# pyranha-labs/hypergrep

Measured on AMD Instinct MI355X. Metric: GiB/s scanned (256 patterns, 32 GiB synthetic log per GPU, text resident in HBM), higher is better.
Workload: dtype u8

## Files before the change

__graft_entry__.py:

```python
from __future__ import annotations

import os
import subprocess
import sys

REPO = os.path.dirname(os.path.abspath(__file__))
if REPO not in sys.path:
    sys.path.insert(0, REPO)


def build() -> None:
    try:
        import torch
    except ImportError:
        pass
    from hypergrep_amd import build as native

    native.build(verbose=bool(os.environ.get("HG_VERBOSE")))
    subprocess.check_call(["make", "-C", os.path.join(REPO, "oracle")], stdout=subprocess.DEVNULL)
    sys.path.insert(0, os.path.join(REPO, "tests"))
    import hgsim_py

    hgsim_py.build()
    import hypergrep_amd

    assert hypergrep_amd.check_compatibility(["foobar"]) == 0


def smoke() -> None:
    import torch

    sys.path.insert(0, os.path.join(REPO, "tests"))
    import oracle_py
    from hypergrep_amd import benchspec, device

    assert torch.cuda.is_available(), "smoke() needs a GPU"
    patterns, needles, hpm = benchspec.c3_spec()
    nbytes = 4 << 20
# ... 20 lines not shown
```

hypergrep_amd/csrc/hg_compile.cpp:

```cpp
#include "hg_compile.h"
#include "hg_comb.h"
#include "hg_core.h"

#include <algorithm>
#include <array>
#include <bitset>
#include <cmath>
#include <cstdlib>
#include <cstring>
#include <map>
#include <memory>
#include <stdexcept>
#include <unordered_map>

namespace {

using ByteSet = std::bitset<256>;

constexpr int kThisExpression = -2;
struct CompileError : std::runtime_error {
  int index;
  explicit CompileError(const std::string &what, int index = kThisExpression) : std::runtime_error(what), index(index) {}
};

// ... 931 lines not shown
Lit clip(const Lit &l, size_t *offset = nullptr) {
  if (offset) *offset = 0;
  if (l.bytes.size() <= HG_FACTOR_MAX) return l;
  size_t best = 0;
  int best_score = INT32_MAX;
  for (size_t o = 0; o + HG_FACTOR_MAX <= l.bytes.size(); o++) {
    int s = 0;
    for (size_t i = 0; i < HG_FACTOR_MAX; i++) s += byte_commonness(static_cast<unsigned char>(l.bytes[o + i]));
    if (s < best_score) { best_score = s; best = o; }
  }
  if (offset) *offset = best;
  return {l.bytes.substr(best, HG_FACTOR_MAX), l.cmask.substr(best, HG_FACTOR_MAX)};
}

struct SampleStats {
  std::unordered_map<uint32_t, uint32_t> c4;
  std::unordered_map<uint64_t, uint32_t> c6;
  size_t dwords = 0;
};

int build_filter(HgDb &db, const SampleStats *stats, std::string *err) {
  db.windows.clear();
  std::vector<std::pair<uint32_t, HgWindow>> keyed;
  std::vector<uint32_t> next16_of;
  const uint32_t fold = db.fold_mask;
  const uint32_t wbytes = db.window_bytes, wmask = db.window_mask;
  std::unordered_map<uint32_t, uint32_t> contenders;
  for (uint32_t fi = 0; fi < db.nreal_factors; fi++) {
    const HgFactor &fct = db.factors[fi];
    std::vector<uint32_t> mine;
// ... 226 lines not shown
        if (rate < k_rate) { k_rate = rate; k_w = weights; }
      }
      if (k_rate < best_rate) { best_rate = k_rate; best_k = k; best_w = k_w; }
      if (k_rate <= (k <= 12 ? 5e-4 : 3e-4)) {
        best_rate = k_rate;
        best_k = k;
        best_w = k_w;
        placed = true;
      }
    }
    if (!placed && best_k && best_rate <= 2e-3 && values.size() * 100 <= (size_t(1) << HG_FILTER_MAX_LOG2) * 45) placed = true;
    if (placed) {
      const uint32_t k = best_k, wa = best_w;
      const uint32_t byte_mask = ((1u << k) - 1u) << 2;
      slot_words(k, wa, db.filter);
      db.ext.assign(size_t(1) << k, HgSlotInfo{});
      db.filter_log2 = k;
      db.weights_a = wa;
      db.weights_b = wa;
      auto merge = [](uint32_t &val, uint32_t &mask, uint32_t v2, uint32_t m2) {
        uint32_t keep = 0;
        for (int b = 0; b < 4; b++) {
          uint32_t bm = 0xFFu << (8 * b);
          if ((mask & bm) && (m2 & bm) && ((val ^ v2) & bm) == 0) keep |= bm;
        }
        mask = keep;
        val &= keep;
      };
      for (size_t wi = 0; wi < keyed.size(); wi++) {
        const HgWindow &w = keyed[wi].second;
// ... 69 lines not shown
      for (size_t e = 0; e < entries.size() && placed; e++) {
        int32_t cur = static_cast<int32_t>(e);
        bool ok = false;
        for (int kick = 0; kick < 8000 && !ok; kick++) {
          const uint32_t cand[4] = {entries[cur].sa * 2, entries[cur].sa * 2 + 1, entries[cur].sb * 2, entries[cur].sb * 2 + 1};
          for (uint32_t cell : cand)
            if (owner[cell] < 0) { owner[cell] = cur; ok = true; break; }
          if (ok) break;
          rng = rng * 6364136223846793005ull + 1442695040888963407ull;
          std::swap(cur, owner[cand[(rng >> 33) & 3]]);
        }
        if (!ok) placed = false;
      }
      if (!placed) continue;
      db.filter.assign(size_t(1) << k, HG_FILTER_EMPTY);
      for (size_t cell = 0; cell < cells; cell++) {
        if (owner[cell] < 0) continue;
        uint32_t &word = db.filter[cell >> 1];
        const uint32_t fp = entries[owner[cell]].fp;
        word = (cell & 1) ? ((word & 0x0000FFFFu) | (fp << 16)) : ((word & 0xFFFF0000u) | fp);
      }
      db.ext.assign(1, HgSlotInfo{});
      db.filter_log2 = k;
      db.filter_wide = 1;
      db.weights_a = wa;
      db.weights_b = wb;
    }
  }
  if (!placed) {
    if (err) *err = "too many distinct literal windows for the LDS filter (more than ~55 000)";
// ... 867 lines not shown
int hgc_tune(const HgDb *db, const uint8_t *sample, size_t nbytes, HgDb **out, std::string *err) {
  if (out) *out = nullptr;
  if (!db || !out || (!sample && nbytes)) return -1;
  SampleStats st;
  const uint32_t fold = db->fold_mask;
  for (size_t p = 0; p + 4 <= nbytes; p += db->dense ? db->dense : 4) {
    uint32_t w, nx = 0;
    std::memcpy(&w, sample + p, 4);
    if (p + 8 <= nbytes) std::memcpy(&nx, sample + p + 4, 4);
    w = (w | fold) & db->window_mask;
    nx |= fold;
    st.c4[w]++;
    st.c6[static_cast<uint64_t>(w) | (static_cast<uint64_t>(nx & 0xFFFFu) << 32)]++;
  }
  st.dwords = nbytes / 4;
  std::unique_ptr<HgDb> copy;
  try {
    copy = std::make_unique<HgDb>(*db);
  } catch (const std::bad_alloc &) {
    if (err) *err = "out of memory";
    return -2;
  }
  int rc = build_filter(*copy, &st, err);
  if (rc != 0) return rc;
  copy->tuned = true;
  *out = copy.release();
  return 0;
}

void hgc_free(HgDb *db) { delete db; }
// ... 1 lines not shown
```

hypergrep_amd/csrc/hg_compile.h:

```cpp
#pragma once
#include <cstdint>
#include <string>
#include <vector>

#include "../../include/hypergrep_amd.h"
#include "hg_core.h"
#include "hg_db.h"

struct HgDb {
  std::vector<HgPattern> patterns;
  std::vector<uint32_t> pool;
  std::vector<HgFactor> factors;
  uint32_t nreal_factors = 0;
  std::vector<HgWindow> windows;
  std::vector<uint32_t> bucket_off;
  std::vector<uint16_t> disc;
  std::vector<uint32_t> bucket_off2;
  std::vector<HgWindow> windows2;
  std::vector<HgWinBucket> wtab;
  uint32_t wtab_mask = 0;
  uint32_t shared_windows = 0;
  uint32_t wtab_first = 0;
  std::vector<uint32_t> filter;
  uint32_t filter_log2 = HG_FILTER_MIN_LOG2;
  uint32_t filter_wide = 0;
  uint32_t window_bytes = HG_WINDOW_BYTES;
  uint32_t window_mask = HG_WINDOW_MASK;
  uint32_t weights_c = HG_HASH_WEIGHTS;
  uint32_t dense = 0;
  uint32_t weights_a = HG_SLOT_WEIGHT_CHOICES[0][0], weights_b = HG_SLOT_WEIGHT_CHOICES[0][1];
  std::vector<HgSlotInfo> ext;
  std::vector<uint32_t> slow;
  uint32_t nslow_fast = 0;
  std::vector<HgSlowGroup> groups;
  uint32_t nslow_grouped = 0;
  uint32_t fold_mask = 0;
  uint32_t max_nw = 1;
  uint32_t nhuge = 0;
// ... 26 lines not shown
```

hypergrep_amd/csrc/hg_db.h:

```cpp
#pragma once
#include <cstdint>

#if defined(__HIPCC__)
#define HG_HD __host__ __device__ __forceinline__
#else
#define HG_HD inline
#endif

constexpr uint32_t HG_FLAG_CASELESS = 1, HG_FLAG_DOTALL = 2, HG_FLAG_MULTILINE = 4, HG_FLAG_SINGLEMATCH = 8;
constexpr uint32_t HG_FLAG_SOM_LEFTMOST = 256;
constexpr uint32_t HG_FLAG_COMBINATION = 512, HG_FLAG_QUIET = 1024;
constexpr uint32_t HG_FLAGS_SUPPORTED = 15 | HG_FLAG_SOM_LEFTMOST | HG_FLAG_COMBINATION | HG_FLAG_QUIET;

enum : uint32_t { HG_PC_START = 0, HG_PC_NL = 1, HG_PC_WORD = 2, HG_PC_OTHER = 3 };
enum : uint32_t { HG_NC_NL = 0, HG_NC_NLFINAL = 1, HG_NC_WORD = 2, HG_NC_OTHER = 3, HG_NC_END = 4 };
constexpr uint32_t HG_TT_ALL = (1u << 20) - 1;

constexpr uint32_t HG_MAX_NODES = 1024;
constexpr uint32_t HG_MAX_W = HG_MAX_NODES / 32;
constexpr uint32_t HG_HUGE_MAX_PROGRAM = 400000;
constexpr uint32_t HG_HUGE_MAX_NODES = 1u << 19;
constexpr uint32_t HG_HUGE_STAGE_MAX = 12288;
constexpr uint32_t HG_HUGE_MAX_EDGES = 1u << 22;
constexpr uint32_t HG_MAX_PATTERNS = 1u << 24;
// ... 127 lines not shown
  uint32_t ctx_off;
  uint32_t reserved;
};
static_assert(sizeof(HgSlowGroup) == 104, "HgSlowGroup layout");

HG_HD uint32_t hg_dot4(uint32_t v, uint32_t w) {
#if defined(__HIP_DEVICE_COMPILE__)
  return __builtin_amdgcn_udot4(v, w, 0u, false);
#else
  return (v & 0xff) * (w & 0xff) + ((v >> 8) & 0xff) * ((w >> 8) & 0xff) + ((v >> 16) & 0xff) * ((w >> 16) & 0xff) + (v >> 24) * (w >> 24);
#endif
}
HG_HD uint32_t hg_hash_window(uint32_t folded) { return hg_dot4(folded, HG_HASH_WEIGHTS); }
HG_HD uint32_t hg_slot(uint32_t folded, uint32_t weights, uint32_t byte_mask) { return hg_dot4(folded, weights) & byte_mask; }
HG_HD bool hg_slot_match(uint32_t slot_word, uint32_t hash_c) { return (hash_c & (slot_word >> 16)) == (slot_word & 0xFFFFu); }
HG_HD uint32_t hg_slot_wide(uint32_t sum_x, uint32_t sum_y, uint32_t byte_mask) { return (sum_x + (sum_y << 8)) & byte_mask; }

struct HgFilterExt {
  uint32_t pv, pm;
  uint32_t nv, nm;
};
HG_HD bool hg_ext_pass(const HgFilterExt &e, uint32_t prev_folded, uint32_t next_folded) {
  return (((prev_folded ^ e.pv) & e.pm) | ((next_folded ^ e.nv) & e.nm)) == 0;
}

constexpr uint32_t HG_DISC_WEIGHTS_1 = 0xc5a36b1du, HG_DISC_WEIGHTS_2 = 0x3b9d47e1u;
HG_HD uint32_t hg_disc_bytes(uint32_t sel4) {
  return ((sel4 & 1u) ? 0xFFu : 0u) | ((sel4 & 2u) ? 0xFF00u : 0u) | ((sel4 & 4u) ? 0xFF0000u : 0u) | ((sel4 & 8u) ? 0xFF000000u : 0u);
}
HG_HD uint32_t hg_disc_bucket(uint32_t h, uint32_t masked_dword) {
// ... 26 lines not shown
```

hypergrep_amd/csrc/hg_engine.h:

```cpp
#pragma once
#include <hip/hip_runtime.h>

#include <memory>
#include <string>

#include "../../include/hypergrep_amd.h"
#include "hg_compile.h"
#include "hg_core.h"
#include "hg_invert.h"
#include "hg_post.h"

#ifndef HG_STREAM_WG_WAVES
#define HG_STREAM_WG_WAVES 8
#endif
constexpr uint32_t HG_STREAM_WG_WAVES_DEFAULT = HG_STREAM_WG_WAVES;

constexpr uint32_t HG_CONFIRM_SPLIT = 4;
constexpr uint32_t HG_DEFER_SHARDS = 64;

struct HgDeferred {
  uint64_t pos;
  uint32_t pattern;
  uint32_t rank;
};
enum { HG_ST_MINLEN_KEPT = 16, HG_ST_FIN_TOTAL = 24, HG_ST_SELECTED = 28, HG_ST_FINAL = 32, HG_ST_WORDS = 36, HG_ST_ZERO_WORDS = 32,
       HG_ST_BLOCK_DONE = 40 };
enum { HG_CNT_CANDS = 0, HG_CNT_HITS = 1, HG_CNT_CAND_NEED = 2, HG_CNT_HIT_NEED = 3, HG_CNT_DEFER_NEED = 4,
       HG_CNT_HITS_WRAPPED = 5,
       HG_CNT_JOIN_TILES = 6,
       HG_CNT_WORDS = 8,
       HG_CNT_CURSOR0 = 64,
       HG_CNT_CURSORS = 64,
       HG_ST_ALLOC_WORDS = 128 };
constexpr uint32_t HG_STREAM_GRAB = 2 * HG_STREAM_WG_WAVES_DEFAULT;

constexpr uint32_t HG_FIN_MAX_BUCKETS = 1u << 22;
constexpr uint32_t HG_FIN_BUCKET_CAP = 4096;
constexpr uint32_t HG_FIN_MEDIUM_CAP = 512;

#ifndef HG_CONFIRM_THREADS
#define HG_CONFIRM_THREADS 128
#endif



// ... 237 lines not shown
```

hypergrep_amd/csrc/hg_engine.hip:

```cpp
#include <algorithm>
#include <array>
#include <cstdio>
#include <cstdlib>
#include <cstring>
#include <memory>

#include "hg_engine.h"
#include "hg_mem.h"

#include <rocprim/rocprim.hpp>

bool hg_launch_stream(const HgStreamArgs &a, uint32_t grid, hipStream_t stream);
bool hg_launch_stream_join(const HgStreamArgs &a, uint32_t grid, hipStream_t stream);
int hg_stream_blocks_per_cu(uint32_t filter_log2, uint32_t filter_wide, uint32_t dense);
__global__ void hg_tile_reduce_kernel(const HgTileSum *sums, uint64_t tile_begin, uint64_t tile_end, uint64_t bs1, HgTileElem *agg);
__global__ void hg_tile_spine_kernel(const HgTileElem *agg, uint32_t nblocks, uint64_t bs1, HgTileBase *block_base, HgTileBase *state);
__global__ void hg_tile_apply_kernel(const HgTileSum *sums, uint64_t tile_begin, uint64_t tile_end, uint64_t bs1, const HgTileBase *block_base,
                                     HgTileBase *bases);
__global__ void hg_tile_inner_kernel(const uint8_t *text, HgTileSum *sums, uint64_t tile_begin, uint64_t tile_end, uint64_t bs1);
__global__ void hg_verify_kernel(HgConfirmArgs a);
__global__ void hg_confirm_fast_kernel(HgConfirmArgs a, uint32_t blocks_per_mode);
__global__ void hg_confirm_generic_kernel(HgConfirmArgs a);
__global__ void hg_always_on_kernel(HgConfirmArgs a, uint32_t first, uint32_t last);
__global__ void hg_always_on_fast_kernel(HgConfirmArgs a);
// ... 118 lines not shown
  knobs_ = HgEngineKnobs::from_env();
  const HgDb &db = *db_;
  HG_TRY(hipSetDevice(device_), "hipSetDevice");
  hipDeviceProp_t prop;
  HG_TRY(hipGetDeviceProperties(&prop, device_), "hipGetDeviceProperties");
  num_cus_ = prop.multiProcessorCount;
  HG_TRY(upload(&d_patterns_, db.patterns, "d_patterns_"), "upload patterns");
  HG_TRY(upload(&d_pool_, db.pool, "d_pool_"), "upload tables");
  HG_TRY(upload(&d_factors_, db.factors, "d_factors_"), "upload factors");
  HG_TRY(upload(&d_windows_, db.windows, "d_windows_"), "upload windows");
  HG_TRY(upload(&d_bucket_, db.bucket_off, "d_bucket_"), "upload buckets");
  HG_TRY(upload(&d_disc_, db.disc, "d_disc_"), "upload discriminators");
  HG_TRY(upload(&d_bucket2_, db.bucket_off2, "d_bucket2_"), "upload buckets");
  HG_TRY(upload(&d_windows2_, db.windows2, "d_windows2_"), "upload windows");
  HG_TRY(upload(&d_wtab_, db.wtab, "d_wtab_"), "upload window table");
  HG_TRY(upload(&d_filter_, db.filter, "d_filter_"), "upload filter");
  HG_TRY(upload(&d_ext_, db.ext, "d_ext_"), "upload filter conditions");
  HG_TRY(upload(&d_slow_, db.slow, "d_slow_"), "upload always-on list");
  HG_TRY(upload(&d_groups_, db.groups, "d_groups_"), "upload always-on groups");
  view_.patterns = static_cast<const HgPattern *>(d_patterns_);
  view_.pool = static_cast<const uint32_t *>(d_pool_);
  view_.factors = static_cast<const HgFactor *>(d_factors_);
  view_.windows = static_cast<const HgWindow *>(d_windows_);
  view_.bucket_off = static_cast<const uint32_t *>(d_bucket_);
  view_.disc = static_cast<const uint16_t *>(d_disc_);
  view_.bucket_off2 = static_cast<const uint32_t *>(d_bucket2_);
  view_.windows2 = static_cast<const HgWindow *>(d_windows2_);
  view_.wtab = static_cast<const HgWinBucket *>(d_wtab_);
  view_.wtab_mask = db.wtab_mask;
  view_.wtab_first = db.wtab_first;
  view_.slow = static_cast<const uint32_t *>(d_slow_);
// ... 214 lines not shown
    p.wgs_alone = knobs_.stream_wgs_per_cu ? p.wgs_shared : grid_for(static_cast<uint32_t>(stream_wgs_per_cu_));
    p.joiner_wgs = (p.piped && stream_wgs_per_cu_ >= 3 && per_cu < static_cast<uint32_t>(stream_wgs_per_cu_) && chunk_limit_tiles_ == 0 && !side_bound_) ? static_cast<uint32_t>(num_cus_) : 0u;
    if (knobs_.joiner >= 0) p.joiner_wgs = p.piped ? static_cast<uint32_t>(knobs_.joiner) * static_cast<uint32_t>(num_cus_) : 0u;
    if (p.wgs_shared + p.joiner_wgs > max_segs_ || db_->filter_wide || db_->filter_log2 > 13) p.joiner_wgs = 0;
    p.wgs = std::max(p.wgs_shared + p.joiner_wgs, p.wgs_alone);
    for (uint32_t c = 0; c < std::min(nchunks, 2u); c++)
      p.cand_seg_cap[c] = static_cast<uint32_t>(static_cast<uint64_t>(cand_cap_) * 4 / (4ull * p.wgs_of(c) + p.joiners_of(c)));
  }
  HgStreamArgs &sa = p.sa;
  sa.text = text;
  sa.nbytes = nbytes;
  sa.db = view_;
  sa.filter = static_cast<const uint32_t *>(d_filter_);
  sa.filter_log2 = db_->filter_log2;
  sa.weights_a = db_->weights_a;
  sa.weights_b = db_->weights_b;
  sa.filter_wide = db_->filter_wide;
  sa.dense = db_->dense;
  sa.weights_c = db_->weights_c;
  sa.ext = static_cast<const HgSlotInfo *>(d_ext_);
  sa.sums = d_sums_;
  sa.counters = d_counters_;
  HgConfirmArgs &ca = p.ca;
  ca.text = text;
  ca.nbytes = nbytes;
  ca.bs1 = bs1;
  ca.db = view_;
  ca.sums = d_sums_;
  ca.bases = d_bases_;
  ca.hits = d_hits_raw_;
  ca.aux = d_aux_raw_;
// ... 437 lines not shown
  HG_TRY(hipMemcpyAsync(h_counters_, d_counters_, HG_ST_WORDS * 4, hipMemcpyDeviceToHost, stream), "copy state");
  if (p.bucketed) HG_TRY(hipEventRecord(ev_[3], stream), "event");
  HG_TRY(hipStreamSynchronize(stream), "stream sync (scan kernels)");
  if (p.piped) {
    uint32_t late = 0;
    for (uint32_t c = 0; c < p.nchunks; c++) {
      float ms = 0;
      (void)hipEventElapsedTime(&ms, ev_k1_begin_[c], ev_k1_end_[c]);
      out->ms_stream += ms;
      if (c >= 1 && hipEventElapsedTime(&ms, ev_k1_end_[c], ev_side_done_[c - 1]) == hipSuccess && ms > 0) late++;
    }
    side_bound_ = late * 2 > p.nchunks - 1;
  }

  out->joiner_tiles = h_counters_[HG_CNT_JOIN_TILES];
  const uint64_t n_raw = p.bucketed ? h_counters_[HG_ST_FIN_TOTAL + 1] : h_counters_[HG_CNT_HITS];
  if (int rc = regrow(p, n_raw)) return rc;
  fin_expect_hits_ = n_raw;
  const uint64_t n_pieces = block_mode ? 1 : !range.last ? 0 : h_final_->L - line_base + (nbytes > h_final_->cs ? hg_pieces(nbytes - h_final_->cs, bs1) : 0);
  uint32_t n = static_cast<uint32_t>(n_raw);
  const HgHit *fin_hits = d_hits_raw_;
  const HgHitAux *fin_aux = d_aux_raw_;
  if (n && d_min_lengths_) {
    if (int rc = minlen_pass(text, &n, p.stream)) return rc;
    fin_hits = d_minlen_hits_;
    fin_aux = d_minlen_aux_;
  }
  if (n && !p.bucketed)
    if (int rc = finalize_compact(fin_hits, fin_aux, n, p.id_bits, p.to_bits, line_base + (range.last ? n_pieces : nbytes) + 1, p.stream)) return rc;
  if (!p.bucketed) {
// ... 150 lines not shown
```

hypergrep_amd/csrc/hg_stream.hip:

```cpp
#include <hip/hip_runtime.h>
#include <cstdlib>

#include "hg_core.h"
#include "hg_engine.h"

namespace {

constexpr int WG_WAVES = HG_STREAM_WG_WAVES;
constexpr int WG_THREADS = WG_WAVES * 64;
constexpr int ITERS = HG_TILE_BYTES / 1024;

__device__ __forceinline__ uint32_t wave_inclusive_scan(uint32_t v, uint32_t lane) {
#pragma unroll
  for (int o = 1; o < 64; o <<= 1) {
    uint32_t u = __shfl_up(v, o, 64);
    if (lane >= static_cast<uint32_t>(o)) v += u;
  }
  return v;
}

}

namespace {

// ... 15 lines not shown
using lds_u32 = __attribute__((address_space(3))) uint32_t;

constexpr uint32_t queue_cap(int) { return 128u; }
constexpr bool queue_stash(int log2, bool dense) { return log2 <= 12 && !dense; }
constexpr uint32_t queue_entry_dw(int log2, bool dense) { return queue_stash(log2, dense) ? 8u : 2u; }
__device__ __forceinline__ uint32_t queue_chunk(uint32_t e0) { return e0 >> 16; }
__device__ __forceinline__ uint32_t queue_rank(uint32_t e0) { return e0 & 0xFFFFu; }

template <int LOG2, bool WIDE>
struct Probe {
  static constexpr uint32_t BYTE_MASK = ((1u << LOG2) - 1u) << 2;
  __device__ __forceinline__ static uint32_t at(const lds_u32 *filter, uint32_t byte_off) {
    return *reinterpret_cast<const lds_u32 *>(reinterpret_cast<const __attribute__((address_space(3))) uint8_t *>(filter) + byte_off);
  }
  template <bool ANY_ONLY, bool FOLD = true>
  __device__ __forceinline__ static uint32_t probe4(const lds_u32 *filter, uint32_t fold, uint32_t wa, uint32_t wb, uint4 v) {
    const uint32_t f0 = FOLD ? v.x | fold : v.x, f1 = FOLD ? v.y | fold : v.y, f2 = FOLD ? v.z | fold : v.z, f3 = FOLD ? v.w | fold : v.w;
    const uint32_t a0 = hg_dot4(f0, wa), a1 = hg_dot4(f1, wa), a2 = hg_dot4(f2, wa), a3 = hg_dot4(f3, wa);
    const uint32_t b0 = hg_dot4(f0, wb), b1 = hg_dot4(f1, wb), b2 = hg_dot4(f2, wb), b3 = hg_dot4(f3, wb);
    const uint32_t c0 = hg_dot4(f0, HG_HASH_WEIGHTS), c1 = hg_dot4(f1, HG_HASH_WEIGHTS);
    const uint32_t c2 = hg_dot4(f2, HG_HASH_WEIGHTS), c3 = hg_dot4(f3, HG_HASH_WEIGHTS);
    if (WIDE) {
      auto wide = [&](uint32_t x, uint32_t y) { return at(filter, hg_slot_wide(x, y, BYTE_MASK)); };
      const uint32_t ta0 = wide(a0, b0), tb0 = wide(b0, a0), ta1 = wide(a1, b1), tb1 = wide(b1, a1);
      const uint32_t ta2 = wide(a2, b2), tb2 = wide(b2, a2), ta3 = wide(a3, b3), tb3 = wide(b3, a3);
      auto m = [](uint32_t t, uint32_t c) { return static_cast<uint16_t>(t) == static_cast<uint16_t>(c) || static_cast<uint16_t>(t >> 16) == static_cast<uint16_t>(c); };
      const bool m0 = m(ta0, c0) || m(tb0, c0), m1 = m(ta1, c1) || m(tb1, c1), m2 = m(ta2, c2) || m(tb2, c2), m3 = m(ta3, c3) || m(tb3, c3);
      if (ANY_ONLY) return (m0 || m1 || m2 || m3) ? 1u : 0u;
      return (m0 ? 1u : 0u) | (m1 ? 2u : 0u) | (m2 ? 4u : 0u) | (m3 ? 8u : 0u);
    }
    const uint32_t t0 = at(filter, a0 & BYTE_MASK), t1 = at(filter, a1 & BYTE_MASK), t2 = at(filter, a2 & BYTE_MASK), t3 = at(filter, a3 & BYTE_MASK);
    const bool m0 = hg_slot_match(t0, c0), m1 = hg_slot_match(t1, c1), m2 = hg_slot_match(t2, c2), m3 = hg_slot_match(t3, c3);
    if (ANY_ONLY) return (m0 || m1 || m2 || m3) ? 1u : 0u;
    return (m0 ? 1u : 0u) | (m1 ? 2u : 0u) | (m2 ? 4u : 0u) | (m3 ? 8u : 0u);
  }
  template <bool FOLD>
  __device__ __forceinline__ static bool any4(const lds_u32 *filter, uint32_t fold, uint32_t wa, uint32_t wb, uint4 v, uint64_t &mask) {
    if (WIDE) {
      const bool any = probe4<true, FOLD>(filter, fold, wa, wb, v) != 0;
      mask = __builtin_amdgcn_ballot_w64(any);
      return any;
    }
    const uint32_t f0 = FOLD ? v.x | fold : v.x, f1 = FOLD ? v.y | fold : v.y, f2 = FOLD ? v.z | fold : v.z, f3 = FOLD ? v.w | fold : v.w;
    const uint32_t a0 = hg_dot4(f0, wa), a1 = hg_dot4(f1, wa), a2 = hg_dot4(f2, wa), a3 = hg_dot4(f3, wa);
    const uint32_t t0 = at(filter, a0 & BYTE_MASK), t1 = at(filter, a1 & BYTE_MASK), t2 = at(filter, a2 & BYTE_MASK), t3 = at(filter, a3 & BYTE_MASK);
    const uint32_t c0 = hg_dot4(f0, HG_HASH_WEIGHTS), c1 = hg_dot4(f1, HG_HASH_WEIGHTS);
    const uint32_t c2 = hg_dot4(f2, HG_HASH_WEIGHTS), c3 = hg_dot4(f3, HG_HASH_WEIGHTS);
    const bool m0 = hg_slot_match(t0, c0), m1 = hg_slot_match(t1, c1), m2 = hg_slot_match(t2, c2), m3 = hg_slot_match(t3, c3);
    mask = __builtin_amdgcn_ballot_w64(m0) | __builtin_amdgcn_ballot_w64(m1) | __builtin_amdgcn_ballot_w64(m2) | __builtin_amdgcn_ballot_w64(m3);
    return m0 || m1 || m2 || m3;
  }
};

template <int LOG2, int STEP>
struct ProbeBytes {
  static constexpr uint32_t BYTE_MASK = ((1u << LOG2) - 1u) << 2;
  template <bool ANY_ONLY>
  __device__ __forceinline__ static uint32_t probe16(const lds_u32 *filter, uint32_t fold, uint32_t wa, uint32_t wc, uint4 v, uint32_t nxt) {
    const uint32_t d[5] = {v.x | fold, v.y | fold, v.z | fold, v.w | fold, nxt | fold};
    uint32_t bits = 0;
#pragma unroll
    for (int j = 0; j < 4; j++) {
      uint32_t w[4], t[4];
      w[0] = d[j];
#pragma unroll
// ... 36 lines not shown

struct StreamCtx {
  const uint4 *text16;
  uint64_t nbytes;
  const lds_u32 *filter;
  const HgSlotInfo *ext;
  lds_u32 *queue;
  lds_u32 *cand_count;
  HgCand *seg;
  uint32_t seg_cap, fold, wa, wb;
};

#if defined(__HIP_DEVICE_COMPILE__)
static_assert(sizeof(StreamCtx) <= 64, "StreamCtx is passed by value to the out-of-line drain routine: beyond 16 dwords it travels through scratch (measured: 1.1 GB of scratch writes per 8 GiB launch, stream pass 20 % slower)");
#endif

__device__ __forceinline__ uint4 load_chunk_checked(const uint4 *__restrict__ text16, uint64_t nbytes, uint64_t g) {
  uint4 v = make_uint4(0, 0, 0, 0);
  if ((g << 4) < nbytes) {
    v = text16[g];
    const uint64_t byte0 = g << 4;
    if (byte0 + 16 > nbytes) {
      const uint32_t valid = static_cast<uint32_t>(nbytes - byte0);
      uint32_t w[4] = {v.x, v.y, v.z, v.w};
#pragma unroll
      for (int k = 0; k < 4; k++) {
        const uint32_t lo = k * 4u;
        if (valid <= lo) w[k] = 0;
        else if (valid < lo + 4) w[k] &= (1u << ((valid - lo) * 8)) - 1u;
      }
// ... 85 lines not shown
      right = e[3];
      cur = make_uint4(e[4], e[5], e[6], e[7]);
    } else {
      cur = load_chunk_checked(cx.text16, cx.nbytes, g);
      if (!WIDE) {
        const uint32_t *text32 = reinterpret_cast<const uint32_t *>(cx.text16);
        left = g ? text32[g * 4 - 1] : 0u;
        if (((g + 1) << 4) < cx.nbytes) {
          right = text32[g * 4 + 4];
          const uint64_t rest = cx.nbytes - ((g + 1) << 4);
          if (rest < 4) right &= (1u << (rest * 8)) - 1u;
        }
        have_left = have_right = true;
      }
    }
    uint32_t l1 = Probe<LOG2, WIDE>::template probe4<false>(cx.filter, cx.fold, cx.wa, cx.wb, cur);
    if ((g << 4) + 16 > cx.nbytes) l1 &= (g << 4) < cx.nbytes ? (1u << static_cast<uint32_t>((cx.nbytes - (g << 4) + 3) >> 2)) - 1u : 0u;
    if (WIDE) {
      hits = l1;
    } else if (l1) {
      constexpr uint32_t BYTE_MASK = ((1u << LOG2) - 1u) << 2;
      for (uint32_t todo = l1 & 15u; todo; todo &= todo - 1) {
        const uint32_t k = __ffs(todo) - 1;
        const uint32_t wk = k == 0 ? cur.x : (k == 1 ? cur.y : (k == 2 ? cur.z : cur.w));
        const uint32_t wp = k == 0 ? left : (k == 1 ? cur.x : (k == 2 ? cur.y : cur.z));
        const uint32_t wn = k == 0 ? cur.y : (k == 1 ? cur.z : (k == 2 ? cur.w : right));
        const uint32_t f = wk | cx.fold;
        const HgSlotInfo info = cx.ext[(hg_dot4(f, cx.wa) & BYTE_MASK) >> 2];
        const uint32_t pm_keep = (k == 0 && !have_left) ? 0u : 0xFFFFFFFFu;
        const uint32_t nm_keep = (k == 3 && !have_right) ? (HG_WINDOW_BYTES == 4 ? 0u : 0xFFu) : 0xFFFFFFFFu;
        const uint32_t prev = wp | cx.fold;
// ... 13 lines not shown
  }
  uint32_t base = 0;
  if (lane == 0) base = __hip_atomic_fetch_add(cx.cand_count, total, __ATOMIC_RELAXED, __HIP_MEMORY_SCOPE_WORKGROUP);
  base = __builtin_amdgcn_readfirstlane(base);
  const uint64_t pos = g << 4;
#pragma unroll
  for (int k = 0; k < 4; k++) {
    if ((hits >> k) & 1u) {
      const uint32_t s = base + slot[k];
      if (s < cx.seg_cap) cx.seg[s] = HgCand{pos + 4u * k, words[k], rank};
    }
    rank += __popc(~not_newline_bits(words[k]));
  }
}

template <int LOG2, bool WIDE, int DENSE, bool FULL, int DEPTH, bool FOLD>
__device__ __forceinline__ void stream_tile(const StreamCtx &cx, uint64_t tile, HgTileSum *__restrict__ sums, uint32_t lane, uint32_t &qn) {
  const uint4 *__restrict__ text16 = cx.text16;
  const uint64_t nbytes = cx.nbytes;
  const uint64_t chunk0 = tile * (HG_TILE_BYTES / 16) + lane;

  const __amdgpu_buffer_rsrc_t tile_rsrc = __builtin_amdgcn_make_buffer_rsrc(const_cast<uint4 *>(text16 + tile * (HG_TILE_BYTES / 16)), 0, HG_TILE_BYTES, 0x00020000);
  const uint32_t lane_off = lane * 16u;
  auto load_chunk = [&](int it) -> uint4 {
    const uint64_t g = chunk0 + static_cast<uint64_t>(it) * 64u;
    if (FULL) {
      if (WIDE) return text16[g];
      if (DENSE) {
        typedef uint32_t u32x4 __attribute__((ext_vector_type(4)));
        const u32x4 v = __builtin_nontemporal_load(reinterpret_cast<const u32x4 *>(text16) + g);
        return make_uint4(v.x, v.y, v.z, v.w);
      }
// ... 1 lines not shown
      return text16[g];
#else
      typedef uint32_t u32x4 __attribute__((ext_vector_type(4)));
      const u32x4 v = __builtin_amdgcn_raw_buffer_load_b128(tile_rsrc, lane_off, it * 1024, 2);
      return make_uint4(v.x, v.y, v.z, v.w);
#endif
    }
    return load_chunk_checked(text16, nbytes, g);
  };

  uint32_t seen = 0;
  uint32_t first_nl = HG_NONE32, last_nl = HG_NONE32;
  uint32_t first_it = 0, last_it = 0;
  uint64_t first_nlm = 0, last_nlm = 0;
  const uint32_t lane_key = lane << 16;

  auto load_after = [&](int it) -> uint32_t {
    if (!DENSE || lane != 63u) return 0u;
    return load_dword_checked(text16, nbytes, (chunk0 + static_cast<uint64_t>(it) * 64u + 1u) << 4);
  };

  auto body = [&](int it, uint4 cur, uint32_t after) {
    uint32_t notnl = __popc(not_newline_bits(cur.x));
    notnl = popc_add(not_newline_bits(cur.y), notnl);
    notnl = popc_add(not_newline_bits(cur.z), notnl);
    notnl = popc_add(not_newline_bits(cur.w), notnl);
#if defined(HG_ABLATE) && HG_ABLATE == 2
    const uint32_t c = cur.x == 0x0a0a0a0au ? 1u : 0u;
    const bool has_nl = c != 0, several_nl = c > 1;
#else
    const uint32_t c = 128u - notnl;
    const bool has_nl = notnl != 128u, several_nl = notnl < 127u;
#endif

#if defined(HG_ABLATE) && HG_ABLATE == 1
    bool any = (cur.x ^ cur.y ^ cur.z ^ cur.w) == 0x12345678u;
    uint64_t am = __builtin_amdgcn_ballot_w64(any);
#else
    bool any;
    uint64_t am;
    if constexpr (DENSE) {
      const uint32_t nxt = __builtin_amdgcn_update_dpp(after, cur.x, 0x130 , 0xF, 0xF, false);
      any = ProbeBytes<LOG2, DENSE ? DENSE : 1>::template probe16<true>(cx.filter, cx.fold, cx.wa, cx.wb, cur, nxt) != 0;
      am = __builtin_amdgcn_ballot_w64(any);
    } else {
      any = Probe<LOG2, WIDE>::template any4<FOLD>(cx.filter, cx.fold, cx.wa, cx.wb, cur, am);
    }
#endif

    if constexpr (!FULL) {
      any = any && ((chunk0 + static_cast<uint64_t>(it) * 64u) << 4) < nbytes;
      am = __builtin_amdgcn_ballot_w64(any);
    }

    const uint64_t nlm = __builtin_amdgcn_ballot_w64(has_nl);
    const uint64_t multi = __builtin_amdgcn_ballot_w64(several_nl);
    if constexpr (!DENSE) {
      if (nlm && first_nl == HG_NONE32) {
        const uint32_t l = __builtin_ctzll(nlm);
        first_nl = static_cast<uint32_t>(it) * 1024u + l * 16u + (__ffs(newline_bits16(readlane4(cur, l))) - 1);
      }
// ... 6 lines not shown
      first_nlm = first_nlm ? first_nlm : nlm;
    }
    last_it = nlm ? static_cast<uint32_t>(it) : last_it;
    last_nlm = nlm ? nlm : last_nlm;
    const uint32_t key = lane_key + opaque_sgpr(seen + (static_cast<uint32_t>(it) << 22));
    uint32_t total, e0 = 0;
    if (__builtin_expect(multi == 0, 1)) {
      total = __popcll(nlm);
      e0 = __builtin_amdgcn_mbcnt_hi(static_cast<uint32_t>(nlm >> 32), __builtin_amdgcn_mbcnt_lo(static_cast<uint32_t>(nlm), key));
    } else {
      const uint32_t incl = wave_inclusive_scan(c, lane);
      total = __builtin_amdgcn_readlane(incl, 63);
      e0 = key + incl - c;
    }
    if (am) {
      const uint32_t left = __builtin_amdgcn_mov_dpp(cur.w, 0x138 , 0xF, 0xF, true);
      const uint32_t right = __builtin_amdgcn_mov_dpp(cur.x, 0x130 , 0xF, 0xF, true);
      if (any) {
        const uint32_t idx = __builtin_amdgcn_mbcnt_hi(static_cast<uint32_t>(am >> 32), __builtin_amdgcn_mbcnt_lo(static_cast<uint32_t>(am), 0u));
        lds_u32 *e = (cx.queue + qn * queue_entry_dw(LOG2, DENSE)) + idx * queue_entry_dw(LOG2, DENSE);
        e[0] = e0;
        e[1] = static_cast<uint32_t>(tile);
        if (queue_stash(LOG2, DENSE)) {
          e[2] = left;
          e[3] = right;
          e[4] = cur.x;
          e[5] = cur.y;
          e[6] = cur.z;
          e[7] = cur.w;
        }
      }
      qn += __popcll(am);
      if (qn >= queue_cap(LOG2) - 64u) {
        const uint32_t n = qn < 64u ? qn : 64u;
        qn -= n;
        drain_batch<LOG2, WIDE, DENSE>(cx, qn, n, lane);
      }
    }
    seen += total;
  };

  if constexpr (FULL) {
    uint4 buf[DEPTH];
    uint32_t abuf[DEPTH];
#pragma unroll
    for (int d = 0; d < DEPTH; d++) { buf[d] = load_chunk(d); abuf[d] = load_after(d); }
#pragma unroll
// ... 51 lines not shown
  cx.nbytes = nbytes;
  cx.filter = (const lds_u32 *)(&s_mem[0]);
  cx.queue = (lds_u32 *)(&s_mem[FILTER_U4]) + wave * queue_cap(LOG2) * queue_entry_dw(LOG2, DENSE);
  cx.cand_count = (lds_u32 *)(&s_mem[FILTER_U4 + QUEUE_U4]);
  cx.ext = reinterpret_cast<const HgSlotInfo *>(ext16);
  cx.seg = cands + static_cast<uint64_t>(blockIdx.x) * seg_cap;
  cx.seg_cap = seg_cap;
  cx.fold = fold;
  cx.wa = wa;
  cx.wb = wb;
  const uint64_t full_tiles = nbytes >> HG_TILE_SHIFT;
  lds_u32 *s_run = cx.cand_count + 1;
  const uint32_t ntile = static_cast<uint32_t>(tile_end - tile_begin);
  const uint32_t nfull = full_tiles > tile_begin ? static_cast<uint32_t>(full_tiles - tile_begin < ntile ? full_tiles - tile_begin : ntile) : 0u;
  uint32_t qn = 0, joined = 0;
  for (;;) {
    if (threadIdx.x == 0) *s_run = atomicAdd(&counters[cursor_slot], HG_STREAM_GRAB);
    __syncthreads();
    const uint32_t r0 = __builtin_amdgcn_readfirstlane(*s_run);
    __syncthreads();
    if (r0 >= ntile) break;
    const uint32_t r1 = r0 + HG_STREAM_GRAB < ntile ? r0 + HG_STREAM_GRAB : ntile;
    if (JOIN) joined += r1 - r0;
    for (uint32_t r = r0 + wave; r < r1; r += WG_WAVES) {
      if (r < nfull) stream_tile<LOG2, WIDE, DENSE, true, DEPTH, FOLD>(cx, tile_begin + r, sums, lane, qn);
      else stream_tile<LOG2, WIDE, DENSE, false, DEPTH, FOLD>(cx, tile_begin + r, sums, lane, qn);
    }
  }
  if (qn) drain_batch<LOG2, WIDE, DENSE>(cx, 0u, qn, lane);
  __syncthreads();
  if (threadIdx.x == 0) {
    const uint32_t n = *cx.cand_count;
    seg_count[blockIdx.x] = n < seg_cap ? n : seg_cap;
    atomicAdd(&counters[HG_CNT_CANDS], n < seg_cap ? n : seg_cap);
    if (n > seg_cap) atomicMax(&counters[HG_CNT_CAND_NEED], n);
    if (JOIN && joined) atomicAdd(&counters[HG_CNT_JOIN_TILES], joined);
  }
}
template <int LOG2, bool WIDE, int DENSE, int DEPTH, bool FOLD = true>
__global__ __launch_bounds__(WG_THREADS) __attribute__((amdgpu_waves_per_eu(HG_STREAM_WAVES, 8))) void hg_stream_kernel(
    const uint4 *__restrict__ text16, uint64_t nbytes, uint64_t tile_begin, uint64_t tile_end, const uint4 *__restrict__ filter16, const uint4 *__restrict__ ext16, uint32_t fold,
    uint32_t wa, uint32_t wb, HgTileSum *__restrict__ sums, HgCand *__restrict__ cands, uint32_t seg_cap, uint32_t *__restrict__ seg_count, uint32_t *__restrict__ counters,
    uint32_t cursor_slot) {
#ifdef HG_STREAM_PRIO
// ... 147 lines not shown
```

Baseline: 5026.

## Add adjacency-keyed LDS filter to cut false-positive candidate queueing

Builds an alternate filter table whose 16-bit check mixes the window hash with the byte before and after each literal window. The stream kernel can then reject candidates whose neighbours cannot match, fetching left/right dwords via DPP. The compiler enables it only when a sample scan shows it removes enough row hits, and signals it through weights_b. The cost is extra ALU work per probe and DPP moves in the hot loop, plus a weaker fingerprint because some hash bits are now spent on neighbour bytes.

```diff
diff --git a/__graft_entry__.py b/__graft_entry__.py
--- a/__graft_entry__.py
+++ b/__graft_entry__.py
@@ -19,9 +19,11 @@
     native.build(verbose=bool(os.environ.get("HG_VERBOSE")))
     subprocess.check_call(["make", "-C", os.path.join(REPO, "oracle")], stdout=subprocess.DEVNULL)
     sys.path.insert(0, os.path.join(REPO, "tests"))
+    import adjsim_py
     import hgsim_py
 
     hgsim_py.build()
+    adjsim_py.build()
     import hypergrep_amd
 
     assert hypergrep_amd.check_compatibility(["foobar"]) == 0
diff --git a/hypergrep_amd/csrc/hg_compile.cpp b/hypergrep_amd/csrc/hg_compile.cpp
--- a/hypergrep_amd/csrc/hg_compile.cpp
+++ b/hypergrep_amd/csrc/hg_compile.cpp
@@ -969,6 +969,8 @@
 }
 
 struct SampleStats {
+  const uint8_t *sample = nullptr;
+  size_t nbytes = 0;
   std::unordered_map<uint32_t, uint32_t> c4;
   std::unordered_map<uint64_t, uint32_t> c6;
   size_t dwords = 0;
@@ -1225,6 +1227,54 @@
       const uint32_t k = best_k, wa = best_w;
       const uint32_t byte_mask = ((1u << k) - 1u) << 2;
       slot_words(k, wa, db.filter);
+      db.filter_adj.clear();
+      if (!db.dense && wbytes == 4) {
+        db.filter_adj.assign(size_t(1) << k, HG_FILTER_EMPTY);
+        std::vector<uint8_t> used(size_t(1) << k, 0);
+        for (size_t wi = 0; wi < keyed.size(); wi++) {
+          const HgWindow &w = keyed[wi].second;
+          const HgFactor &f = db.factors[w.factor_off >> 8];
+          const uint32_t o = w.factor_off & 0xff;
+          uint32_t prev = 0, next = 0, known = 0;
+          if (o >= 1) {
+            prev = static_cast<uint32_t>(f.lit[o - 1] | (fold & 0xFFu)) << 24;
+            known |= (!fold && hg_factor_cmask(f, o - 1) != 0xFF) ? 0x00DFu : 0x00FFu;
+          }
+          if (o + wbytes + 1 <= f.len) {
+            next = static_cast<uint32_t>(f.lit[o + wbytes] | (fold & 0xFFu));
+            known |= (!fold && hg_factor_cmask(f, o + wbytes) != 0xFF) ? 0xDF00u : 0xFF00u;
+          }
+          const uint32_t key = hg_adj_key(hg_hash_window(w.value), prev, next) & 0xFFFFu;
+          uint32_t &word = db.filter_adj[hg_slot(w.value, wa, byte_mask) >> 2];
+          if (!used[hg_slot(w.value, wa, byte_mask) >> 2]) {
+            word = (known << 16) | (key & known);
+            used[hg_slot(w.value, wa, byte_mask) >> 2] = 1;
+          } else {
+            const uint32_t care = (word >> 16) & known & ~((word ^ key) & 0xFFFFu);
+            word = (care << 16) | (word & care);
+          }
+        }
+      }
+      if (!db.filter_adj.empty() && stats && stats->sample && stats->nbytes >= 1024) {
+        auto dword_at = [&](size_t p) {
+          uint32_t x = 0;
+          std::memcpy(&x, stats->sample + p, std::min<size_t>(4, stats->nbytes - p));
+          return x | fold;
+        };
+        size_t rows = 0, rows_old = 0, rows_adj = 0;
+        for (size_t row = 0; row + 1024 <= stats->nbytes; row += 1024, rows++) {
+          bool any_old = false, any_adj = false;
+          for (size_t p = row; p < row + 1024; p += 4) {
+            const uint32_t v = dword_at(p), sl = hg_slot(v, wa, byte_mask) >> 2, c = hg_hash_window(v);
+            any_old = any_old || hg_slot_match(db.filter[sl], c);
+            const uint32_t keep = p == row ? HG_ADJ_KEEP_NO_PREV : (p == row + 1020 ? HG_ADJ_KEEP_NO_NEXT : HG_ADJ_KEEP_ALL);
+            any_adj = any_adj || hg_slot_miss(db.filter_adj[sl], c, p >= 4 ? dword_at(p - 4) : 0u, p + 4 < stats->nbytes ? dword_at(p + 4) : 0u, keep) == 0;
+          }
+          rows_old += any_old;
+          rows_adj += any_adj;
+        }
+        if (rows_old < rows_adj || (rows_old - rows_adj) * 3 < rows) db.filter_adj.clear();
+      }
       db.ext.assign(size_t(1) << k, HgSlotInfo{});
       db.filter_log2 = k;
       db.weights_a = wa;
@@ -1324,6 +1374,7 @@
       }
       if (!placed) continue;
       db.filter.assign(size_t(1) << k, HG_FILTER_EMPTY);
+      db.filter_adj.clear();
       for (size_t cell = 0; cell < cells; cell++) {
         if (owner[cell] < 0) continue;
         uint32_t &word = db.filter[cell >> 1];
@@ -2221,6 +2272,8 @@
     st.c6[static_cast<uint64_t>(w) | (static_cast<uint64_t>(nx & 0xFFFFu) << 32)]++;
   }
   st.dwords = nbytes / 4;
+  st.sample = sample;
+  st.nbytes = nbytes;
   std::unique_ptr<HgDb> copy;
   try {
     copy = std::make_unique<HgDb>(*db);
diff --git a/hypergrep_amd/csrc/hg_compile.h b/hypergrep_amd/csrc/hg_compile.h
--- a/hypergrep_amd/csrc/hg_compile.h
+++ b/hypergrep_amd/csrc/hg_compile.h
@@ -22,6 +22,7 @@
   uint32_t shared_windows = 0;
   uint32_t wtab_first = 0;
   std::vector<uint32_t> filter;
+  std::vector<uint32_t> filter_adj;
   uint32_t filter_log2 = HG_FILTER_MIN_LOG2;
   uint32_t filter_wide = 0;
   uint32_t window_bytes = HG_WINDOW_BYTES;
diff --git a/hypergrep_amd/csrc/hg_db.h b/hypergrep_amd/csrc/hg_db.h
--- a/hypergrep_amd/csrc/hg_db.h
+++ b/hypergrep_amd/csrc/hg_db.h
@@ -165,6 +165,12 @@
 HG_HD uint32_t hg_hash_window(uint32_t folded) { return hg_dot4(folded, HG_HASH_WEIGHTS); }
 HG_HD uint32_t hg_slot(uint32_t folded, uint32_t weights, uint32_t byte_mask) { return hg_dot4(folded, weights) & byte_mask; }
 HG_HD bool hg_slot_match(uint32_t slot_word, uint32_t hash_c) { return (hash_c & (slot_word >> 16)) == (slot_word & 0xFFFFu); }
+static_assert(HG_WINDOW_BYTES == 4, "hg_slot_miss takes the byte after the window from byte 0 of the next dword: 4-byte windows only");
+constexpr uint32_t HG_ADJ_KEEP_ALL = 0xFFFFu, HG_ADJ_KEEP_NO_PREV = 0xFF00u, HG_ADJ_KEEP_NO_NEXT = 0x00FFu;
+HG_HD uint32_t hg_adj_key(uint32_t hash_c, uint32_t prev, uint32_t next) { return hash_c ^ ((next << 8) | (prev >> 24)); }
+HG_HD uint32_t hg_slot_miss(uint32_t slot_word, uint32_t hash_c, uint32_t prev, uint32_t next, uint32_t keep) {
+  return (hg_adj_key(hash_c, prev, next) ^ slot_word) & (slot_word >> 16) & keep;
+}
 HG_HD uint32_t hg_slot_wide(uint32_t sum_x, uint32_t sum_y, uint32_t byte_mask) { return (sum_x + (sum_y << 8)) & byte_mask; }
 
 struct HgFilterExt {
diff --git a/hypergrep_amd/csrc/hg_engine.h b/hypergrep_amd/csrc/hg_engine.h
--- a/hypergrep_amd/csrc/hg_engine.h
+++ b/hypergrep_amd/csrc/hg_engine.h
@@ -29,6 +29,7 @@
        HG_CNT_HITS_WRAPPED = 5,
        HG_CNT_JOIN_TILES = 6,
        HG_CNT_WORDS = 8,
+       HG_CNT_STREAM_AM_ITERS = 8, HG_CNT_STREAM_QUEUED = 9, HG_CNT_STREAM_DRAINS = 10,
        HG_CNT_CURSOR0 = 64,
        HG_CNT_CURSORS = 64,
        HG_ST_ALLOC_WORDS = 128 };
diff --git a/hypergrep_amd/csrc/hg_engine.hip b/hypergrep_amd/csrc/hg_engine.hip
--- a/hypergrep_amd/csrc/hg_engine.hip
+++ b/hypergrep_amd/csrc/hg_engine.hip
@@ -156,7 +156,7 @@
   HG_TRY(upload(&d_bucket2_, db.bucket_off2, "d_bucket2_"), "upload buckets");
   HG_TRY(upload(&d_windows2_, db.windows2, "d_windows2_"), "upload windows");
   HG_TRY(upload(&d_wtab_, db.wtab, "d_wtab_"), "upload window table");
-  HG_TRY(upload(&d_filter_, db.filter, "d_filter_"), "upload filter");
+  HG_TRY(upload(&d_filter_, db.filter_adj.empty() ? db.filter : db.filter_adj, "d_filter_"), "upload filter");
   HG_TRY(upload(&d_ext_, db.ext, "d_ext_"), "upload filter conditions");
   HG_TRY(upload(&d_slow_, db.slow, "d_slow_"), "upload always-on list");
   HG_TRY(upload(&d_groups_, db.groups, "d_groups_"), "upload always-on groups");
@@ -401,7 +401,7 @@
   sa.filter = static_cast<const uint32_t *>(d_filter_);
   sa.filter_log2 = db_->filter_log2;
   sa.weights_a = db_->weights_a;
-  sa.weights_b = db_->weights_b;
+  sa.weights_b = db_->filter_wide ? db_->weights_b : (db_->filter_adj.empty() ? 0u : 1u);
   sa.filter_wide = db_->filter_wide;
   sa.dense = db_->dense;
   sa.weights_c = db_->weights_c;
@@ -869,6 +869,10 @@
   }
 
   out->joiner_tiles = h_counters_[HG_CNT_JOIN_TILES];
+#if defined(HG_STREAM_COUNTS)
+  fprintf(stderr, "stream counts: bytes %llu queued_chunks %u am_iterations %u drain_calls %u candidates %u\n", static_cast<unsigned long long>(nbytes),
+          h_counters_[HG_CNT_STREAM_QUEUED], h_counters_[HG_CNT_STREAM_AM_ITERS], h_counters_[HG_CNT_STREAM_DRAINS], h_counters_[HG_CNT_CANDS]);
+#endif
   const uint64_t n_raw = p.bucketed ? h_counters_[HG_ST_FIN_TOTAL + 1] : h_counters_[HG_CNT_HITS];
   if (int rc = regrow(p, n_raw)) return rc;
   fin_expect_hits_ = n_raw;
diff --git a/hypergrep_amd/csrc/hg_stream.hip b/hypergrep_amd/csrc/hg_stream.hip
--- a/hypergrep_amd/csrc/hg_stream.hip
+++ b/hypergrep_amd/csrc/hg_stream.hip
@@ -1,3 +1,4 @@
+#include <type_traits>
 #include <hip/hip_runtime.h>
 #include <cstdlib>
 
@@ -53,7 +54,8 @@
     return *reinterpret_cast<const lds_u32 *>(reinterpret_cast<const __attribute__((address_space(3))) uint8_t *>(filter) + byte_off);
   }
   template <bool ANY_ONLY, bool FOLD = true>
-  __device__ __forceinline__ static uint32_t probe4(const lds_u32 *filter, uint32_t fold, uint32_t wa, uint32_t wb, uint4 v) {
+  __device__ __forceinline__ static uint32_t probe4(const lds_u32 *filter, uint32_t fold, uint32_t wa, uint32_t wb, uint4 v, bool adj = false, uint32_t left = 0,
+                                                    uint32_t right = 0, uint32_t keep_left = HG_ADJ_KEEP_ALL, uint32_t keep_right = HG_ADJ_KEEP_ALL) {
     const uint32_t f0 = FOLD ? v.x | fold : v.x, f1 = FOLD ? v.y | fold : v.y, f2 = FOLD ? v.z | fold : v.z, f3 = FOLD ? v.w | fold : v.w;
     const uint32_t a0 = hg_dot4(f0, wa), a1 = hg_dot4(f1, wa), a2 = hg_dot4(f2, wa), a3 = hg_dot4(f3, wa);
     const uint32_t b0 = hg_dot4(f0, wb), b1 = hg_dot4(f1, wb), b2 = hg_dot4(f2, wb), b3 = hg_dot4(f3, wb);
@@ -69,12 +71,22 @@
       return (m0 ? 1u : 0u) | (m1 ? 2u : 0u) | (m2 ? 4u : 0u) | (m3 ? 8u : 0u);
     }
     const uint32_t t0 = at(filter, a0 & BYTE_MASK), t1 = at(filter, a1 & BYTE_MASK), t2 = at(filter, a2 & BYTE_MASK), t3 = at(filter, a3 & BYTE_MASK);
-    const bool m0 = hg_slot_match(t0, c0), m1 = hg_slot_match(t1, c1), m2 = hg_slot_match(t2, c2), m3 = hg_slot_match(t3, c3);
+    const uint32_t fl = FOLD ? left | fold : left, fr = FOLD ? right | fold : right;
+    bool m0, m1, m2, m3;
+    if (adj) {
+      m0 = hg_slot_miss(t0, c0, fl, f1, keep_left) == 0, m1 = hg_slot_miss(t1, c1, f0, f2, HG_ADJ_KEEP_ALL) == 0;
+      m2 = hg_slot_miss(t2, c2, f1, f3, HG_ADJ_KEEP_ALL) == 0, m3 = hg_slot_miss(t3, c3, f2, fr, keep_right) == 0;
+    } else {
+      m0 = hg_slot_match(t0, c0), m1 = hg_slot_match(t1, c1), m2 = hg_slot_match(t2, c2), m3 = hg_slot_match(t3, c3);
+    }
     if (ANY_ONLY) return (m0 || m1 || m2 || m3) ? 1u : 0u;
     return (m0 ? 1u : 0u) | (m1 ? 2u : 0u) | (m2 ? 4u : 0u) | (m3 ? 8u : 0u);
   }
   template <bool FOLD>
-  __device__ __forceinline__ static bool any4(const lds_u32 *filter, uint32_t fold, uint32_t wa, uint32_t wb, uint4 v, uint64_t &mask) {
+  __device__ __forceinline__ static uint32_t folded(uint32_t fold, uint32_t d) { return FOLD ? d | fold : d; }
+  template <bool FOLD, bool ADJ = false>
+  __device__ __forceinline__ static bool any4(const lds_u32 *filter, uint32_t fold, uint32_t wa, uint32_t wb, uint4 v, uint64_t &mask, uint32_t left = 0, uint32_t right = 0,
+                                              uint32_t keep_left = HG_ADJ_KEEP_ALL, uint32_t keep_right = HG_ADJ_KEEP_ALL) {
     if (WIDE) {
       const bool any = probe4<true, FOLD>(filter, fold, wa, wb, v) != 0;
       mask = __builtin_amdgcn_ballot_w64(any);
@@ -85,9 +97,17 @@
     const uint32_t t0 = at(filter, a0 & BYTE_MASK), t1 = at(filter, a1 & BYTE_MASK), t2 = at(filter, a2 & BYTE_MASK), t3 = at(filter, a3 & BYTE_MASK);
     const uint32_t c0 = hg_dot4(f0, HG_HASH_WEIGHTS), c1 = hg_dot4(f1, HG_HASH_WEIGHTS);
     const uint32_t c2 = hg_dot4(f2, HG_HASH_WEIGHTS), c3 = hg_dot4(f3, HG_HASH_WEIGHTS);
-    const bool m0 = hg_slot_match(t0, c0), m1 = hg_slot_match(t1, c1), m2 = hg_slot_match(t2, c2), m3 = hg_slot_match(t3, c3);
-    mask = __builtin_amdgcn_ballot_w64(m0) | __builtin_amdgcn_ballot_w64(m1) | __builtin_amdgcn_ballot_w64(m2) | __builtin_amdgcn_ballot_w64(m3);
-    return m0 || m1 || m2 || m3;
+    if (!ADJ) {
+      const bool m0 = hg_slot_match(t0, c0), m1 = hg_slot_match(t1, c1), m2 = hg_slot_match(t2, c2), m3 = hg_slot_match(t3, c3);
+      mask = __builtin_amdgcn_ballot_w64(m0) | __builtin_amdgcn_ballot_w64(m1) | __builtin_amdgcn_ballot_w64(m2) | __builtin_amdgcn_ballot_w64(m3);
+      return m0 || m1 || m2 || m3;
+    }
+    const uint32_t r0 = hg_slot_miss(t0, c0, left, f1, keep_left), r1 = hg_slot_miss(t1, c1, f0, f2, HG_ADJ_KEEP_ALL);
+    const uint32_t r2 = hg_slot_miss(t2, c2, f1, f3, HG_ADJ_KEEP_ALL), r3 = hg_slot_miss(t3, c3, f2, right, keep_right);
+    const uint32_t r01 = r0 < r1 ? r0 : r1, r23 = r2 < r3 ? r2 : r3;
+    const bool any = (r01 < r23 ? r01 : r23) == 0;
+    mask = __builtin_amdgcn_ballot_w64(any);
+    return any;
   }
 };
 
@@ -154,6 +174,12 @@
 #if defined(__HIP_DEVICE_COMPILE__)
 static_assert(sizeof(StreamCtx) <= 64, "StreamCtx is passed by value to the out-of-line drain routine: beyond 16 dwords it travels through scratch (measured: 1.1 GB of scratch writes per 8 GiB launch, stream pass 20 % slower)");
 #endif
+
+struct StreamCounts {
+  uint32_t am_iters = 0;
+  uint32_t queued = 0;
+  uint32_t drains = 0;
+};
 
 __device__ __forceinline__ uint4 load_chunk_checked(const uint4 *__restrict__ text16, uint64_t nbytes, uint64_t g) {
   uint4 v = make_uint4(0, 0, 0, 0);
@@ -269,7 +295,8 @@
         have_left = have_right = true;
       }
     }
-    uint32_t l1 = Probe<LOG2, WIDE>::template probe4<false>(cx.filter, cx.fold, cx.wa, cx.wb, cur);
+    uint32_t l1 = Probe<LOG2, WIDE>::template probe4<false>(cx.filter, cx.fold, cx.wa, cx.wb, cur, !WIDE && !DENSE && cx.wb != 0, left, right, have_left ? HG_ADJ_KEEP_ALL : HG_ADJ_KEEP_NO_PREV,
+                                                            have_right ? HG_ADJ_KEEP_ALL : HG_ADJ_KEEP_NO_NEXT);
     if ((g << 4) + 16 > cx.nbytes) l1 &= (g << 4) < cx.nbytes ? (1u << static_cast<uint32_t>((cx.nbytes - (g << 4) + 3) >> 2)) - 1u : 0u;
     if (WIDE) {
       hits = l1;
@@ -313,8 +340,8 @@
   }
 }
 
-template <int LOG2, bool WIDE, int DENSE, bool FULL, int DEPTH, bool FOLD>
-__device__ __forceinline__ void stream_tile(const StreamCtx &cx, uint64_t tile, HgTileSum *__restrict__ sums, uint32_t lane, uint32_t &qn) {
+template <int LOG2, bool WIDE, int DENSE, bool FULL, int DEPTH, bool FOLD, bool ADJ>
+__device__ __forceinline__ void stream_tile(const StreamCtx &cx, uint64_t tile, HgTileSum *__restrict__ sums, uint32_t lane, uint32_t &qn, StreamCounts &counts) {
   const uint4 *__restrict__ text16 = cx.text16;
   const uint64_t nbytes = cx.nbytes;
   const uint64_t chunk0 = tile * (HG_TILE_BYTES / 16) + lane;
@@ -346,6 +373,7 @@
   uint32_t first_it = 0, last_it = 0;
   uint64_t first_nlm = 0, last_nlm = 0;
   const uint32_t lane_key = lane << 16;
+  const uint32_t keep_left = lane == 0u ? HG_ADJ_KEEP_NO_PREV : HG_ADJ_KEEP_ALL, keep_right = lane == 63u ? HG_ADJ_KEEP_NO_NEXT : HG_ADJ_KEEP_ALL;
 
   auto load_after = [&](int it) -> uint32_t {
     if (!DENSE || lane != 63u) return 0u;
@@ -365,6 +393,7 @@
     const bool has_nl = notnl != 128u, several_nl = notnl < 127u;
 #endif
 
+    uint32_t left = 0, right = 0;
 #if defined(HG_ABLATE) && HG_ABLATE == 1
     bool any = (cur.x ^ cur.y ^ cur.z ^ cur.w) == 0x12345678u;
     uint64_t am = __builtin_amdgcn_ballot_w64(any);
@@ -375,8 +404,12 @@
       const uint32_t nxt = __builtin_amdgcn_update_dpp(after, cur.x, 0x130 , 0xF, 0xF, false);
       any = ProbeBytes<LOG2, DENSE ? DENSE : 1>::template probe16<true>(cx.filter, cx.fold, cx.wa, cx.wb, cur, nxt) != 0;
       am = __builtin_amdgcn_ballot_w64(any);
+    } else if constexpr (!ADJ) {
+      any = Probe<LOG2, WIDE>::template any4<FOLD>(cx.filter, cx.fold, cx.wa, cx.wb, cur, am);
     } else {
-      any = Probe<LOG2, WIDE>::template any4<FOLD>(cx.filter, cx.fold, cx.wa, cx.wb, cur, am);
+      left = __builtin_amdgcn_mov_dpp(Probe<LOG2, WIDE>::template folded<FOLD>(cx.fold, cur.w), 0x138 , 0xF, 0xF, true);
+      right = __builtin_amdgcn_mov_dpp(Probe<LOG2, WIDE>::template folded<FOLD>(cx.fold, cur.x), 0x130 , 0xF, 0xF, true);
+      any = Probe<LOG2, WIDE>::template any4<FOLD, true>(cx.filter, cx.fold, cx.wa, cx.wb, cur, am, left, right, keep_left, keep_right);
     }
 #endif
 
@@ -413,8 +446,10 @@
       e0 = key + incl - c;
     }
     if (am) {
-      const uint32_t left = __builtin_amdgcn_mov_dpp(cur.w, 0x138 , 0xF, 0xF, true);
-      const uint32_t right = __builtin_amdgcn_mov_dpp(cur.x, 0x130 , 0xF, 0xF, true);
+      if constexpr (!ADJ) {
+        left = __builtin_amdgcn_mov_dpp(cur.w, 0x138 , 0xF, 0xF, true);
+        right = __builtin_amdgcn_mov_dpp(cur.x, 0x130 , 0xF, 0xF, true);
+      }
       if (any) {
         const uint32_t idx = __builtin_amdgcn_mbcnt_hi(static_cast<uint32_t>(am >> 32), __builtin_amdgcn_mbcnt_lo(static_cast<uint32_t>(am), 0u));
         lds_u32 *e = (cx.queue + qn * queue_entry_dw(LOG2, DENSE)) + idx * queue_entry_dw(LOG2, DENSE);
@@ -430,6 +465,11 @@
         }
       }
       qn += __popcll(am);
+#if defined(HG_STREAM_COUNTS)
+      counts.am_iters++;
+      counts.queued += __popcll(am);
+      counts.drains += qn >= queue_cap(LOG2) - 64u ? 1u : 0u;
+#endif
       if (qn >= queue_cap(LOG2) - 64u) {
         const uint32_t n = qn < 64u ? qn : 64u;
         qn -= n;
@@ -511,20 +551,37 @@
   const uint32_t ntile = static_cast<uint32_t>(tile_end - tile_begin);
   const uint32_t nfull = full_tiles > tile_begin ? static_cast<uint32_t>(full_tiles - tile_begin < ntile ? full_tiles - tile_begin : ntile) : 0u;
   uint32_t qn = 0, joined = 0;
-  for (;;) {
-    if (threadIdx.x == 0) *s_run = atomicAdd(&counters[cursor_slot], HG_STREAM_GRAB);
-    __syncthreads();
-    const uint32_t r0 = __builtin_amdgcn_readfirstlane(*s_run);
-    __syncthreads();
-    if (r0 >= ntile) break;
-    const uint32_t r1 = r0 + HG_STREAM_GRAB < ntile ? r0 + HG_STREAM_GRAB : ntile;
-    if (JOIN) joined += r1 - r0;
-    for (uint32_t r = r0 + wave; r < r1; r += WG_WAVES) {
-      if (r < nfull) stream_tile<LOG2, WIDE, DENSE, true, DEPTH, FOLD>(cx, tile_begin + r, sums, lane, qn);
-      else stream_tile<LOG2, WIDE, DENSE, false, DEPTH, FOLD>(cx, tile_begin + r, sums, lane, qn);
-    }
+  StreamCounts counts;
+  auto draw = [&](auto adj) {
+    constexpr bool ADJ = decltype(adj)::value;
+    for (;;) {
+      if (threadIdx.x == 0) *s_run = atomicAdd(&counters[cursor_slot], HG_STREAM_GRAB);
+      __syncthreads();
+      const uint32_t r0 = __builtin_amdgcn_readfirstlane(*s_run);
+      __syncthreads();
+      if (r0 >= ntile) break;
+      const uint32_t r1 = r0 + HG_STREAM_GRAB < ntile ? r0 + HG_STREAM_GRAB : ntile;
+      if (JOIN) joined += r1 - r0;
+      for (uint32_t r = r0 + wave; r < r1; r += WG_WAVES) {
+        if (r < nfull) stream_tile<LOG2, WIDE, DENSE, true, DEPTH, FOLD, ADJ>(cx, tile_begin + r, sums, lane, qn, counts);
+        else stream_tile<LOG2, WIDE, DENSE, false, DEPTH, FOLD, ADJ>(cx, tile_begin + r, sums, lane, qn, counts);
+      }
+    }
+  };
+  if constexpr (!WIDE && !DENSE) {
+    if (wb != 0) draw(std::true_type{});
+    else draw(std::false_type{});
+  } else {
+    draw(std::false_type{});
   }
   if (qn) drain_batch<LOG2, WIDE, DENSE>(cx, 0u, qn, lane);
+#if defined(HG_STREAM_COUNTS)
+  if (lane == 0) {
+    atomicAdd(&counters[HG_CNT_STREAM_AM_ITERS], counts.am_iters);
+    atomicAdd(&counters[HG_CNT_STREAM_QUEUED], counts.queued);
+    atomicAdd(&counters[HG_CNT_STREAM_DRAINS], counts.drains + (qn ? 1u : 0u));
+  }
+#endif
   __syncthreads();
   if (threadIdx.x == 0) {
     const uint32_t n = *cx.cand_count;
```

New measurement: 5147 (median of 6 runs). +2.4%, better.
